# BurnhamG/PyTorch-ScalableFHVAE

Hardware: AMD Instinct MI355X
Metric: segments/sec + ELBO (nats/frame), (B,20,80) fbank (higher is better)
Workload: dtype bf16; 1 GPU; c3: fhvae.FHVAE 2x256 LSTM enc/dec, z1=z2=32, 28k-seq mu2 table, batch 2048; per-GPU batch 2048, T=20, F=80, full train step (fwd+loss+bwd+Adam), intended objective, mu_idx uniform; global_batch=2048, parallelism=single

## Files before the change

### pytorch-scalablefhvae_amd/csrc/wgrad.hip

```cpp
#include "wgrad.h"

#include <algorithm>
#include <cstdlib>
#include <type_traits>
#include <vector>

#include "gemm_core.h"

namespace fh {

constexpr int kWgThreads = 512, kWgBM = 256, kMaxWgProblems = FHVAE_WGRAD_MAX_PROBLEMS;

struct WgBf16 {
  using T = u16;
  using Frag = bf16x8;
  static constexpr int BK = 64, KB = 32;
  static constexpr bool kSetprio = true;
  static constexpr unsigned kOob = 0x40000000u;
  static constexpr int64_t kMaxBytes = 1LL << 30;
  static constexpr double kRate = 1.0e15;
  static __device__ __forceinline__ int swizzle(int pc, int row) { return (((pc >> 1) ^ (row & 7)) << 1) | (pc & 1); }
  static constexpr int kXor = 7, kSegShift = 5;
  static __device__ __forceinline__ int krow(int gq, int i) { return 4 * gq + (i >> 2); }
  static __device__ __forceinline__ int sub(int i) { return 8 * (i & 3); }
  template <int RB>
  static __device__ __forceinline__ Frag read(const char* a0) {
    typedef s16x4 __attribute__((address_space(3))) * lds_p;
    union {
      struct {
        s16x4 lo, hi;
      } s;
      bf16x8 v;
    } u;
    u.s.lo = __builtin_amdgcn_ds_read_tr16_b64_v4i16((lds_p)(a0));
    u.s.hi = __builtin_amdgcn_ds_read_tr16_b64_v4i16((lds_p)(a0 + 16 * RB));
    return u.v;
  }
  static __device__ __forceinline__ f32x4 mfma(Frag a, Frag b, f32x4 c) { return __builtin_amdgcn_mfma_f32_16x16x32_bf16(a, b, c, 0, 0, 0); }
};

struct WgF32 {
  using T = float;
  using Frag = float;
  static constexpr int BK = 32, KB = 4;
  static constexpr bool kSetprio = false;
  static constexpr unsigned kOob = 0x7ffffff0u;
  static constexpr int64_t kMaxBytes = 0x7ffffff0LL;
  static constexpr double kRate = 140.0e12;
  static __device__ __forceinline__ int swizzle(int pc, int row) { return (((pc >> 2) ^ (row & 3)) << 2) | (pc & 3); }
  static constexpr int kXor = 3, kSegShift = 6;
  static __device__ __forceinline__ int krow(int gq, int i) { return gq; }
  static __device__ __forceinline__ int sub(int i) { return i * 4; }
  template <int RB>
  static __device__ __forceinline__ Frag read(const char* a0) {
    return *(const float*)a0;
  }
  static __device__ __forceinline__ f32x4 mfma(Frag a, Frag b, f32x4 c) { return __builtin_amdgcn_mfma_f32_16x16x4f32(a, b, c, 0, 0, 0); }
};
template <class T>
using WgElem = std::conditional_t<std::is_same<T, u16>::value, WgBf16, WgF32>;

template <class E>
struct WgGroupT {
  int n;
  int base[kMaxWgProblems + 1];
  WgProblemT<typename E::T> p[kMaxWgProblems];
};

template <class E, int W>
struct WgImg {
  static constexpr int RB = W * (int)sizeof(typename E::T);
  static constexpr int BYTES = E::BK * RB;
  static constexpr int CPR = RB / 16;
  static constexpr int RPI = 1024 / RB;
  static constexpr int NI = BYTES / 1024 / 8;
};

typedef void __attribute__((address_space(3))) * lds_void_p;

template <class E, int W, int NI>
__device__ __forceinline__ void wg_dma_offsets(unsigned (&voff)[NI], unsigned ld_bytes, int wave, int lane) {
  using I = WgImg<E, W>;
#pragma unroll
  for (int q = 0; q < I::NI; ++q) {
    const int row = (wave * I::NI + q) * I::RPI + lane / I::CPR;
    const int pc = lane % I::CPR;
    voff[q] = (unsigned)row * ld_bytes + (unsigned)E::swizzle(pc, row) * 16u;
  }
}

template <class E, int W, int NI>
__device__ __forceinline__ void wg_issue(char* stage, __amdgpu_buffer_rsrc_t rs, const unsigned (&voff)[NI], unsigned kbase, int wave) {
  using I = WgImg<E, W>;
#pragma unroll
  for (int q = 0; q < I::NI; ++q)
    __builtin_amdgcn_raw_ptr_buffer_load_lds(rs, (lds_void_p)(stage + (wave * I::NI + q) * 1024), 16, voff[q] + kbase, 0, 0, 0);
}

template <class E, int BN>
__global__ __launch_bounds__(kWgThreads) void wgrad_kernel(WgGroupT<E> g) {
  using T = typename E::T;
  using IA = WgImg<E, kWgBM>;
  using IB = WgImg<E, BN>;
  constexpr int STAGE = IA::BYTES + IB::BYTES;
  constexpr int TM = 8, TN = BN / 64;
  constexpr int BK = E::BK, NJ = BK / E::KB;
  __shared__ __attribute__((aligned(1024))) char stage0[STAGE];
  __shared__ __attribute__((aligned(1024))) char stage1[STAGE];

  int wg = blockIdx.x;
  {
    const int nb = gridDim.x;
    if (nb >= 16) {
      const int q = nb >> 3, r = nb & 7, xcd = wg & 7;
      wg = (xcd < r ? xcd * (q + 1) : r * (q + 1) + (xcd - r) * q) + (wg >> 3);
    }
  }
  int pi = 0;
  while (pi + 1 < g.n && wg >= g.base[pi + 1]) ++pi;
  const WgProblemT<T>& p = g.p[pi];
  const int local = wg - g.base[pi];
  const int mt = local % p.m_tiles, nt = (local / p.m_tiles) % p.n_tiles, sp = local / (p.m_tiles * p.n_tiles);
  const int ks_total = (p.K + BK - 1) / BK;
  const int ks0 = sp * p.ksteps_per, ks1 = min(ks_total, ks0 + p.ksteps_per);
  if (ks0 >= ks1) return;
  const int m0 = mt * kWgBM, n0 = nt * BN;

  const int tid = threadIdx.x, lane = tid & 63, wave = tid >> 6;
  const int wm = wave >> 2, wn = wave & 3;
  const int gq = lane >> 4, i = lane & 15;

  constexpr unsigned ES = sizeof(T);
  const unsigned lda_b = (unsigned)p.lda * ES, ldb_b = (unsigned)p.ldb * ES;
  const __amdgpu_buffer_rsrc_t rsa =
      __builtin_amdgcn_make_buffer_rsrc(const_cast<T*>(p.A + m0), 0, (int)(((int64_t)p.K * p.lda - p.a_col0 - m0) * ES), 0x00020000);
  const __amdgpu_buffer_rsrc_t rsb =
      __builtin_amdgcn_make_buffer_rsrc(const_cast<T*>(p.B + n0), 0, (int)(((int64_t)p.K * p.ldb - n0) * ES), 0x00020000);
  unsigned va[IA::NI], vb[IB::NI];
  wg_dma_offsets<E, kWgBM>(va, lda_b, wave, lane);
  wg_dma_offsets<E, BN>(vb, ldb_b, wave, lane);

  const int kr = E::krow(gq, i), x = kr & E::kXor;
  int offa[TM], offb[TN];
#pragma unroll
  for (int tm = 0; tm < TM; ++tm) offa[tm] = kr * IA::RB + (((wm * 8 + tm) ^ x) << E::kSegShift) + E::sub(i);
#pragma unroll
  for (int tn = 0; tn < TN; ++tn) offb[tn] = kr * IB::RB + (((wn * TN + tn) ^ x) << E::kSegShift) + E::sub(i);

  f32x4 acc[TM][TN];
#pragma unroll
  for (int tm = 0; tm < TM; ++tm)
#pragma unroll
    for (int tn = 0; tn < TN; ++tn) acc[tm][tn] = f32x4{0.f, 0.f, 0.f, 0.f};

  auto kofs = [&](int ks, unsigned ld_b) __attribute__((always_inline)) -> unsigned { return (unsigned)(ks * BK) * ld_b; };
  auto compute = [&](const char* As, char* nxt, int ks_next) __attribute__((always_inline)) {
    const char* Bs = As + IA::BYTES;
#pragma unroll
    for (int j = 0; j < NJ; ++j) {
      typename E::Frag a[TM], b[TN];
#pragma unroll
      for (int tn = 0; tn < TN; ++tn) b[tn] = E::template read<IB::RB>(Bs + offb[tn] + j * E::KB * IB::RB);
#pragma unroll
      for (int tm = 0; tm < TM; ++tm) a[tm] = E::template read<IA::RB>(As + offa[tm] + j * E::KB * IA::RB);
      if (j == 0 || j == NJ / 2) {
        const bool in = ks_next < ks1;
        if (j == 0)
          wg_issue<E, kWgBM>(nxt, rsa, va, in ? kofs(ks_next, lda_b) : E::kOob, wave);
        else
          wg_issue<E, BN>(nxt + IA::BYTES, rsb, vb, in ? kofs(ks_next, ldb_b) : E::kOob, wave);
      }
      if (E::kSetprio) __builtin_amdgcn_s_setprio(1);
#pragma unroll
      for (int tm = 0; tm < TM; ++tm)
#pragma unroll
        for (int tn = 0; tn < TN; ++tn) acc[tm][tn] = E::mfma(a[tm], b[tn], acc[tm][tn]);
      if (E::kSetprio) __builtin_amdgcn_s_setprio(0);
    }
  };
  auto step = [&](const char* cur, char* nxt, int ks_next) __attribute__((always_inline)) {
    asm volatile("s_waitcnt vmcnt(0)" ::: "memory");
    __builtin_amdgcn_s_barrier();
    compute(cur, nxt, ks_next);
    __builtin_amdgcn_s_barrier();
  };
  wg_issue<E, kWgBM>(stage0, rsa, va, kofs(ks0, lda_b), wave);
  wg_issue<E, BN>(stage0 + IA::BYTES, rsb, vb, kofs(ks0, ldb_b), wave);
  for (int ks = ks0; ks < ks1; ks += 2) {
    step(stage0, stage1, ks + 1);
    step(stage1, stage0, ks + 2);
  }
  asm volatile("s_waitcnt vmcnt(0)" ::: "memory");

#pragma unroll
  for (int tm = 0; tm < TM; ++tm)
#pragma unroll
    for (int tn = 0; tn < TN; ++tn) {
      const int n = n0 + wn * (BN / 4) + tn * 16 + i;
#pragma unroll
      for (int r = 0; r < 4; ++r) {
        const int m = m0 + wm * 128 + tm * 16 + 4 * gq + r;
        if (m < p.M && n < p.N) {
          float* c = p.C + (int64_t)m * p.ldc + n;
          if (p.splitk == 1 && !p.shared_c)
            *c += acc[tm][tn][r];
          else
            atomicAdd(c, acc[tm][tn][r]);
        }
      }
    }
}

template __global__ void wgrad_kernel<WgBf16, 256>(WgGroupT<WgBf16>);
template __global__ void wgrad_kernel<WgBf16, 128>(WgGroupT<WgBf16>);
template __global__ void wgrad_kernel<WgF32, 256>(WgGroupT<WgF32>);
template __global__ void wgrad_kernel<WgF32, 128>(WgGroupT<WgF32>);

template <class T>
bool wgrad_eligible(const WgProblemT<T>& p) {
  using E = WgElem<T>;
  constexpr int64_t ES = sizeof(T);
  if (p.M <= 0 || p.N <= 0 || p.K <= 0 || !p.A || !p.B || !p.C) return false;
  if ((((uintptr_t)p.A) | ((uintptr_t)p.B)) & 15) return false;
  if ((p.lda % (16 / ES)) || (p.ldb % (16 / ES)) || p.lda < p.a_col0 + p.M || p.ldb < p.N || p.a_col0 < 0) return false;
  if ((int64_t)p.K * p.lda * ES >= E::kMaxBytes || (int64_t)p.K * p.ldb * ES >= E::kMaxBytes) return false;
  return true;
}

template <class T>
static void plan_launch(const WgProblemT<T>* ps, fhvae_wgrad_plan& l) {
  using E = WgElem<T>;
  int64_t tiles = 0, ks_max = 1;
  for (int k = 0; k < l.n; ++k) {
    const WgProblemT<T>& p = ps[l.p[k].which];
    tiles += fh_cdiv(p.M, kWgBM) * fh_cdiv(p.N, l.BN);
    ks_max = std::max<int64_t>(ks_max, fh_cdiv(p.K, E::BK));
  }
  const double t_step = 2.0 * kWgBM * l.BN * E::BK / (E::kRate / 256), tile_bytes = 4.0 * kWgBM * l.BN;
  int64_t sk = 1;
  double best = 1e30;
  for (int64_t c = 1; c <= 64 && c * 2 <= ks_max; ++c) {
    const double waves = (double)fh_cdiv(tiles * c, 256), steps = (double)fh_cdiv(ks_max, c) + 2.0;
    const double t = waves * steps * t_step + (c > 1 ? tiles * c * tile_bytes / 1.3e12 : 0.0);
    if (t < best) best = t, sk = c;
  }
  l.sk = (int)sk;
  for (int k = 0; k < l.n; ++k) {
    auto& q = l.p[k];
    const WgProblemT<T>& p = ps[q.which];
    q.m_tiles = (int)fh_cdiv(p.M, kWgBM);
    q.n_tiles = (int)fh_cdiv(p.N, l.BN);
    const int64_t ks_total = fh_cdiv(p.K, E::BK);
    int64_t s = sk;
    if (s > ks_total / 2) s = ks_total / 2;
    if (s < 1) s = 1;
    q.ksteps_per = (int)fh_cdiv(ks_total, s);
    q.splitk = (int)fh_cdiv(ks_total, q.ksteps_per);
    l.grid += q.m_tiles * q.n_tiles * q.splitk;
    for (int b = 0; b < l.n; ++b)
      if (b != k && ps[l.p[b].which].C == p.C) q.shared_c = 1;
  }
}

template <class T>
static int plan_wgrad(const WgProblemT<T>* ps, int n, fhvae_wgrad_plan* out, int cap) {
  if (n > 256) return FHVAE_ERR_LIMIT;
  for (int k = 0; k < n; ++k)
    if (!wgrad_eligible(ps[k])) return FHVAE_ERR_ALIGN;
  int launches = 0;
  for (const int BN : {256, 128}) {
    fhvae_wgrad_plan* l = nullptr;
    for (int k = 0; k < n; ++k) {
      if ((ps[k].N > 128) != (BN == 256)) continue;
// ... 100 lines not shown
```

### pytorch-scalablefhvae_amd/csrc/lstm.hip

```cpp
#include "gemm_launch.h"
#include "lstm_cell.h"
#include "lstm_cluster.h"
#include "lstm_point.h"
#include "wgrad.h"
#include <algorithm>
#include <vector>
#include "trace.h"
#include <cstdlib>
#include <type_traits>

namespace fh {

constexpr int kCH = 32;

struct GateRowMap {
  int H;
  __device__ __forceinline__ int64_t operator()(int n) const {
    int unit = (n >> 6) * 16 + (n & 15);
    int gate = (n & 63) >> 4;
    return unit < H ? (int64_t)gate * H + unit : -1;
  }
  __device__ __forceinline__ bool all_valid(int n0, int n) const { return ((n0 + n) >> 6) * 16 <= H; }
};

// ... 741 lines not shown
  };
  auto wgrad = [&](const void* a, int64_t lda, const void* b, int64_t ldb, int64_t Kc, float* c, int64_t ldc, int64_t Ncols) {
    GemmParams p = {};
    p.seg[0] = Seg{a, lda, 0, b, ldb, 0, (int)Kc, 0};
    p.M = (int)G;
    p.N = (int)Ncols;
    p.C = c;
    p.ldc = ldc;
    p.splitk = 0;
    p.mode = 1;
    return p;
  };
  auto flush = [&]() -> int {
    int e = FHVAE_OK;
    for (int i = 0; i < ng && !e; i += kMaxGroup) e = launch_gemm_group(grp + i, ng - i < kMaxGroup ? ng - i : kMaxGroup, d->dtype, st);
    ng = 0;
    return e;
  };
  for (int l = 0; l < L; ++l) {
    const T* dgl = dg + (int64_t)l * T_ * B * G;
    const T* hl = hs + (int64_t)l * T_ * B * H;
    int e;
    if (bd->dw_hh[l] && T_ > 1 && !wgrad_long(dgl + B * G, G, hl, H, (T_ - 1) * B, bd->dw_hh[l], H, H))
      grp[ng++] = wgrad(dgl + B * G, G, hl, H, (T_ - 1) * B, bd->dw_hh[l], H, H);
    if (bd->dw_ih[l]) {
      if (l > 0) {
        if (!wgrad_long(dgl, G, hs + (int64_t)(l - 1) * T_ * B * H, H, T_ * B, bd->dw_ih[l], H, H))
          grp[ng++] = wgrad(dgl, G, hs + (int64_t)(l - 1) * T_ * B * H, H, T_ * B, bd->dw_ih[l], H, H);
      } else {
        if (I > 0 && !wgrad_long(dgl, G, op.x, I, T_ * B, bd->dw_ih[0], K0, I))
          grp[ng++] = wgrad(dgl, G, op.x, I, T_ * B, bd->dw_ih[0], K0, I);
        if (Ic > 0) {
          GemmParams p = wgrad(bd->dgsum, G, d->xc, Ic, B, bd->dw_ih[0] + I, K0, Ic);
          if (fq) {
            fq->push_back(p);
          } else {
            e = launch_gemm(p, FHVAE_F32, st);
            if (e) return e;
          }
        }
      }
    }
    if (!pl.form) {
      if (l == 0 && Ic > 0 && bd->dgsum)
        e = launch_colsum(bd->dgsum, FHVAE_F32, G, bd->db_ih[l], bd->db_hh[l], B, G, st);
      else
        e = launch_colsum(dgl, d->dtype, G, bd->db_ih[l], bd->db_hh[l], T_ * B, G, st);
      if (e) return e;
    }
  }
  return flush();
}

static int lstm_dxc(const fhvae_lstm_bwd_desc* bd, hipStream_t st, bool zeroed) {
  const fhvae_lstm_desc* d = &bd->f;
  if (!bd->d_xc || d->Ic <= 0) return FHVAE_OK;
  const int64_t G = 4 * d->H, K0 = d->I + d->Ic;
  GemmParams p = {};
  p.seg[0] = Seg{bd->dgsum, G, 1, d->w_ih[0] + d->I, K0, 0, (int)G, 0};
  p.M = (int)d->B;
  p.N = (int)d->Ic;
  p.C = bd->d_xc;
  p.ldc = d->Ic;
  const int64_t tiles = fh_cdiv(d->B, 64) * fh_cdiv(d->Ic, 64);
  if (tiles <= 64 && G >= 512) {
    const int64_t n = d->B * d->Ic;
    if (!zeroed) hipLaunchKernelGGL(zero_f32_kernel, dim3((unsigned)fh_cdiv(n, 1024)), dim3(256), 0, st, bd->d_xc, n);
    p.mode = 2;
    int64_t sk = 256 / tiles;
    while (sk > 1 && G / sk < 128) sk >>= 1;
    p.splitk = (int)(sk < 4 ? 4 : sk > 16 ? 16 : sk);
  } else {
    p.splitk = 1;
  }
  return launch_gemm(p, FHVAE_F32, st);
}

template <typename T>
static int lstm_seq_bwd_t(const fhvae_lstm_bwd_desc* bd, const LstmPlan& pl, const Ops<T>& op, bool rec, bool par, hipStream_t st) {
  int e;
  if (rec) {
    e = lstm_bwd_impl<T>(bd, pl, op, st);
    if (e) return e;
    e = lstm_dxc(bd, st, pl.bwd_zeroes_dxc);
    if (e) return e;
  }
  if (!par) return FHVAE_OK;
  std::vector<WgProblemT<T>> wq;
  e = lstm_param_grads<T>(bd, pl, op, st, &wq);
  if (e) return e;
  return launch_wgrad(wq.data(), (int)wq.size(), st);
}

extern "C" int fhvae_lstm_seq_bwd(const fhvae_lstm_bwd_desc* bd, void* stream) {
  FH_CHECK_PTR(bd);
  const fhvae_lstm_desc* d = &bd->f;
  int e = check_desc(d);
  if (e) return e;
  FH_CHECK_PTR(bd->dgates);
  FH_CHECK_PTR(bd->dc);
  if (d->Ic > 0) FH_CHECK_PTR(bd->dgsum);
  if (bd->phase < 0 || bd->phase > 2) return FHVAE_ERR_SHAPE;
  const bool rec = bd->phase != 2, par = bd->phase != 1;
  if (rec && !bd->d_hs_top && !bd->d_hn) return FHVAE_ERR_NULL;
  hipStream_t st = (hipStream_t)stream;
  const LstmPlan pl = lstm_plan(d);
  if (d->dtype == FHVAE_F32) return lstm_seq_bwd_t<float>(bd, pl, ops_f32(d), rec, par, st);
  return lstm_seq_bwd_t<u16>(bd, pl, ops_bf16(d), rec, par, st);
}

static bool wg_from_desc(const fhvae_wgrad_desc* x, WgProblem& p) {
  if (!x || x->M <= 0 || x->N <= 0 || x->K <= 0 || x->M > INT32_MAX || x->N > INT32_MAX || x->K > INT32_MAX || x->a_col0 < 0 ||
      x->a_col0 > INT32_MAX)
    return false;
  p = WgProblem{};
  p.A = (const u16*)x->a, p.B = (const u16*)x->b, p.C = x->c;
  p.lda = x->lda, p.ldb = x->ldb, p.ldc = x->ldc;
  p.M = (int)x->M, p.N = (int)x->N, p.K = (int)x->K;
  p.a_col0 = (int)x->a_col0;
  return wgrad_eligible(p) && x->ldc >= x->N;
}

extern "C" int fhvae_wgrad_desc_ok(const fhvae_wgrad_desc* x) {
  WgProblem p;
  return wg_from_desc(x, p) ? 1 : 0;
}

extern "C" int fhvae_lstm_param_grads_multi(const fhvae_lstm_bwd_desc* const* bds, int n, const fhvae_wgrad_desc* extra, int n_extra,
                                            void* stream) {
  if (n < 0 || n_extra < 0) return FHVAE_ERR_SHAPE;
  if (n > 0) FH_CHECK_PTR(bds);
  if (n_extra > 0) FH_CHECK_PTR(extra);
  hipStream_t st = (hipStream_t)stream;
  std::vector<WgProblem> wq;
  for (int i = 0; i < n_extra; ++i) {
    WgProblem p;
    if (!wg_from_desc(extra + i, p)) return FHVAE_ERR_ALIGN;
    wq.push_back(p);
  }
  std::vector<GemmParams> fq;
  std::vector<WgProblem32> wq32;
  for (int i = 0; i < n; ++i) {
    const fhvae_lstm_bwd_desc* bd = bds[i];
    FH_CHECK_PTR(bd);
    const fhvae_lstm_desc* d = &bd->f;
    int e = check_desc(d);
    if (e) return e;
    FH_CHECK_PTR(bd->dgates);
    if (d->Ic > 0) FH_CHECK_PTR(bd->dgsum);
    if (d->dtype == FHVAE_F32) {
      e = lstm_param_grads<float>(bd, lstm_plan(d), ops_f32(d), st, &wq32);
    } else {
      e = lstm_param_grads<u16>(bd, lstm_plan(d), ops_bf16(d), st, &wq, &fq);
    }
    if (e) return e;
  }
  for (size_t i = 0; i < fq.size();) {
    size_t j = i;
    while (j < fq.size() && j - i < (size_t)kMaxGroup) {
      bool dup = false;
      for (size_t k = i; k < j; ++k) dup = dup || fq[k].C == fq[j].C;
      if (dup) break;
      ++j;
    }
    const int e = launch_gemm_group(fq.data() + i, (int)(j - i), FHVAE_F32, st);
    if (e) return e;
    i = j;
  }
// ... 7 lines not shown
```

### pytorch-scalablefhvae_amd/csrc/lstm_bwd_rs.hip

```cpp
#include <cstdlib>

#include "lstm_cluster_dev.h"
#include "lstm_point.h"
#include "trace.h"

namespace fh {

namespace {

constexpr int kH = 256, kG = 4 * kH, kHU = 64, kNU = 4;
constexpr int kKS = 8;

template <int RT>
__device__ __forceinline__ int rs_xoff(int par, int cluster, int src, int j, int wave, int rt) {
  return ((((((par * 64 + cluster) * kNU + src) * 3 + (j - 1)) * 4 + wave) * RT + rt) << 9);
}

template <int RT>
struct RsCfg {
  static constexpr int SMEM = RT * 16 * 512;
};

template <int RT, bool UM>
__global__ __launch_bounds__(kThreads) void lstm_bwd_layer_rs_kernel(ClBwd p) {
// ... 138 lines not shown
#pragma unroll
      for (int i = 0; i < 4; ++i) {
        const LstmPointBwd pt = lstm_point_bwd(dh[rt][i], ig[i], fg[i], gg[i], og[i], ccur[rt][i], cprev[rt][i], s > 0, dcreg[rt][i]);
        dcreg[rt][i] = pt.dc;
#pragma unroll
        for (int g = 0; g < 4; ++g) dp[g][i] = pt.dp[g];
      }
      ccur[rt] = cprev[rt];
      const bool live = row[rt] < rend;
#pragma unroll
      for (int g = 0; g < 4; ++g) {
        if (live) dgs[rt][g] += dp[g];
        dpk[rt][g] = pack4(dp[g]);
        *(uint2*)(Img + wbase[g & 1] + (g >> 1) * 256 + rt * 8192) = dpk[rt][g];
      }
    }
    asm volatile("s_waitcnt lgkmcnt(0)\n\ts_barrier" ::: "memory");
    CL_TLOG(s * 8 + 3);
    if (s + 1 < T) {
      f32x4 acc[RT][kNU];
#pragma unroll
      for (int rt = 0; rt < RT; ++rt)
#pragma unroll
        for (int j = 0; j < kNU; ++j) acc[rt][j] = f32x4{0.f, 0.f, 0.f, 0.f};
      bf16x8 bfrag[2][RT];
      auto ifrag = [&](int ks, int buf) {
#pragma unroll
        for (int rt = 0; rt < RT; ++rt)
          bfrag[buf][rt] = __builtin_bit_cast(bf16x8, *(const uint4*)(Img + ibase[ks & 3] + (ks >> 2) * 256 + rt * 8192));
      };
      ifrag(0, 0);
      __builtin_amdgcn_sched_group_barrier(0x100, RT, 0);
#pragma unroll
      for (int ks = 0; ks < kKS; ++ks) {
        if (ks + 1 < kKS) ifrag(ks + 1, (ks + 1) & 1);
#pragma unroll
        for (int j = 0; j < kNU; ++j)
#pragma unroll
          for (int rt = 0; rt < RT; ++rt) acc[rt][j] = __builtin_amdgcn_mfma_f32_16x16x32_bf16(wreg[ks][j], bfrag[ks & 1][rt], acc[rt][j], 0, 0, 0);
        if (ks + 1 < kKS) {
          __builtin_amdgcn_sched_group_barrier(0x008, 1, 0);
          __builtin_amdgcn_sched_group_barrier(0x100, RT, 0);
          __builtin_amdgcn_sched_group_barrier(0x008, RT * kNU - 1, 0);
        } else {
          __builtin_amdgcn_sched_group_barrier(0x008, RT * kNU, 0);
        }
      }
#pragma unroll
      for (int rt = 0; rt < RT; ++rt) {
        own[rt] = acc[rt][0];
#pragma unroll
        for (int j = 1; j < kNU; ++j)
          *(uint2*)((char*)p.xch + rs_xoff<RT>(s & 1, cluster, me, j, wave, rt) + lane * 8) = pack4(acc[rt][j]);
      }
    }
    auto img_chunk = [&](int i) -> uint4 {
      const int c = (wave * RT * 2 + i) * 64 + lane;
      return *(const uint4*)(Img + kc_off<32>(c >> 5, c & 31));
    };
    const uint4 v0 = img_chunk(0), v1 = img_chunk(1), v2 = RT > 1 ? img_chunk(2) : uint4{0u, 0u, 0u, 0u},
                v3 = RT > 1 ? img_chunk(3) : uint4{0u, 0u, 0u, 0u};
    CL_TLOG(s * 8 + 4);
    if (s + 1 < T) cluster_publish(flags, me, ep0 + (unsigned)(s + 1));
    else __syncthreads();
    CL_TLOG(s * 8 + 5);
    auto dg_store = [&](int i, const uint4& v) {
      const int c = (wave * RT * 2 + i) * 64 + lane;
      const int rw = r0 + (c >> 5), cc = c & 31;
      if (rw < rend) {
        u16* dst = p.dg + ((int64_t)t * B + rw) * G + (cc >> 3) * H + u0 + (cc & 7) * 8;
        if (nt)
          __builtin_nontemporal_store(u32x4v{v.x, v.y, v.z, v.w}, (u32x4v*)dst);
        else
          *(uint4*)dst = v;
      }
    };
    dg_store(0, v0);
    dg_store(1, v1);
    if constexpr (RT > 1) {
      dg_store(2, v2);
      dg_store(3, v3);
    }
  }
  if (p.d_xc_zero && me == 0 && wave == 0) {
#pragma unroll
    for (int rt = 0; rt < RT; ++rt)
      if (row[rt] < rend)
        for (int c = q; c < p.Ic; c += 4) p.d_xc_zero[(int64_t)row[rt] * p.Ic + c] = 0.f;
  }
#pragma unroll
  for (int g = 0; g < 4; ++g) {
    f32x4 vs = f32x4{0.f, 0.f, 0.f, 0.f};
#pragma unroll
    for (int rt = 0; rt < RT; ++rt) {
      vs += dgs[rt][g];
      if (p.dgsum && row[rt] < rend) *(f32x4*)(p.dgsum + (int64_t)row[rt] * G + g * H + uq) = dgs[rt][g];
    }
    if (p.db_ih[0] || p.db_hh[0]) db_reduce_add(vs, p.db_ih[0], p.db_hh[0], g * H + uq, lane);
  }
  CL_TLOG((T - 1) * 8 + 7);
}

template <int RT>
int launch_rs(const ClBwd& p, hipStream_t st) {
  if (p.gates_um)
    hipLaunchKernelGGL((lstm_bwd_layer_rs_kernel<RT, true>), dim3(kGrid), dim3(kThreads), RsCfg<RT>::SMEM, st, p);
  else
    hipLaunchKernelGGL((lstm_bwd_layer_rs_kernel<RT, false>), dim3(kGrid), dim3(kThreads), RsCfg<RT>::SMEM, st, p);
  return fh_launch_status();
}

}

int cluster_bwd_layer_rs(const ClBwd& p, hipStream_t st) {
  if (p.NU != kNU || p.Mc > 32 || p.Mc % 16 != 0) return FHVAE_ERR_SHAPE;
  return p.Mc <= 16 ? launch_rs<1>(p, st) : launch_rs<2>(p, st);
}

}
```

### pytorch-scalablefhvae_amd/csrc/lstm_cluster.h

```cpp
#pragma once
#include "common.h"

namespace fh {

constexpr int kSyncStatus = 0;
constexpr int kSyncSticky = 2;
constexpr int kSyncFlags = 64;
constexpr int kSyncXcdCnt = kSyncFlags + 64 * 32;
constexpr int kSyncXcdStride = 32;
constexpr int kSyncWordsUsed = 3072;
constexpr int kSeqEpochs = 4096;

constexpr int64_t kRsXchElems = 2LL * 64 * 4 * 3 * 4 * 2 * 256;

struct ClusterWeights {
  const u16* w_ih[FHVAE_MAX_LAYERS];
  const u16* w_hh[FHVAE_MAX_LAYERS];
  const u16* w_ih_t[FHVAE_MAX_LAYERS];
  const u16* w_hh_t[FHVAE_MAX_LAYERS];
  u16* xch;
  const u16* x_fold;
  const u16* xc_fold;
};

struct LstmPlan {
  int form;
  bool big, big_shape;
  bool fold;
  bool xc_in;
  bool bwd_rs;
  bool fwd_wr;
  bool bwd_zeroes_dxc;
  bool needs_ws_below;
  bool wgrad;
  bool tlog;
  struct Geo {
    int NU, NC;
    int64_t chunk;
  } fwd, bwd;
};
LstmPlan lstm_plan(const fhvae_lstm_desc* d);

int cluster_fwd(const fhvae_lstm_desc* d, const LstmPlan& pl, const ClusterWeights& w, hipStream_t st);
int cluster_bwd(const fhvae_lstm_bwd_desc* bd, const LstmPlan& pl, const ClusterWeights& w, hipStream_t st);

}
```

### pytorch-scalablefhvae_amd/csrc/lstm_cluster.hip

```cpp
#include "lstm_cluster_dev.h"
#include "lstm_point.h"

#include <cstdlib>
#include <cstring>
#include <type_traits>

#include "gemm_core.h"
#include "gemm_launch.h"
#include "proj.h"
#include "trace.h"


namespace fh {

constexpr int kRing = 4;
constexpr int kPanel = 4096;

template <int ROWS, int CH, class RowMap>
__device__ __forceinline__ void glds_wave_panel(char* lds, const u16* base, int64_t ld, int k0, const RowMap& rm, int row_base,
                                                int lane) {
  constexpr int RPI = 64 / CH;
  constexpr int SW = CH >= 16 ? 15 : CH - 1;
  static_assert(ROWS * CH * 16 == kPanel && ROWS % RPI == 0, "panel shape");
#pragma unroll
// ... 1020 lines not shown
        dcreg[i] = pt.dc;
#pragma unroll
        for (int g = 0; g < 4; ++g) dp[g][i] = pt.dp[g];
      }
      ccur = cprev;
      if (row < rend) {
#pragma unroll
        for (int g = 0; g < 4; ++g) dgs[g] += dp[g];
      }
      if (row < rend) {
#pragma unroll
        for (int g = 0; g < 4; ++g) {
          dpk[g] = pack4(dp[g]);
          *(uint2*)(p.xch + xch_off(s & 1, kp, L, KS, (g * H + uq) >> 5, B, row) + (uq & 31)) = dpk[g];
        }
      }
    }
    CL_TLOG(s * 8 + 3);
    if (s + 1 < nsteps) cluster_publish(flags, me, ep0 + (unsigned)(s + 1));
    CL_TLOG(s * 8 + 4);
    if (act && row < rend) {
      u16* go = p.dg + (((int64_t)kp * T + t) * B + row) * G + uq;
#pragma unroll
      for (int g = 0; g < 4; ++g) *(uint2*)(go + g * H) = dpk[g];
    }
  }
  if (p.dgsum && kp == 0 && row < rend) {
#pragma unroll
    for (int g = 0; g < 4; ++g) *(f32x4*)(p.dgsum + (int64_t)row * G + g * H + uq) = dgs[g];
    if (p.d_xc_zero && uq == 0)
      for (int c = 0; c < p.Ic; ++c) p.d_xc_zero[(int64_t)row * p.Ic + c] = 0.f;
  }
  if (epi && (p.db_ih[kp] || p.db_hh[kp])) {
#pragma unroll
    for (int g = 0; g < 4; ++g) db_reduce_add(dgs[g], p.db_ih[kp], p.db_hh[kp], g * H + uq, lane);
  }
}

static bool device_ok() {
  static int ok = -1;
  if (ok < 0) {
    int dev = 0;
    hipDeviceProp_t pr;
    ok = 0;
    if (hipGetDevice(&dev) == hipSuccess && hipGetDeviceProperties(&pr, dev) == hipSuccess)
      ok = (strncmp(pr.gcnArchName, "gfx950", 6) == 0 && pr.multiProcessorCount == kGrid) ? 1 : 0;
  }
  return ok == 1;
}

static void cluster_rows(int64_t nrows, int NC, int* Mc, int* RB) {
  int64_t m = (nrows + NC - 1) / NC;
  m = (m + 15) / 16 * 16;
  *Mc = (int)m;
  *RB = m <= 16 ? 16 : m <= 32 ? 32 : m <= 64 ? 64 : 128;
}

LstmPlan lstm_plan(const fhvae_lstm_desc* d) {
  const int64_t B = d->B, T = d->T, I = d->I, Ic = d->Ic, H = d->H;
  LstmPlan p = {};
  p.wgrad = !getenv("FHVAE_NO_WGRAD");
  const bool persistent = !getenv("FHVAE_NO_CLUSTER") && d->dtype == FHVAE_BF16 && d->lp && (H == 256 || H == 128) && d->L <= 2 &&
                          T + d->L < kSeqEpochs && B <= 131072 &&
                          device_ok();
  if (!persistent) {
    const char* ev = getenv("FHVAE_BIG_CELLS");
    const int want = ev ? atoi(ev) : -1, es = d->dtype == FHVAE_BF16 ? 2 : 4, epc = 16 / es;
    p.big = want >= 0 ? want != 0 : (B / 128) * (H / 64) >= (d->dtype == FHVAE_F32 ? 64 : 96);
    p.big_shape = !(B % 128 || H % 64 || I % epc || Ic % epc) && B * 4 * H * 4 < (1LL << 31) && (int64_t)d->L * H * B * 4 < (1LL << 31) &&
                  4 * H * (I + Ic > H ? I + Ic : H) * es < (1LL << 30);
    return p;
  }
  const int NU = (int)H / 16, NC = kGrid / NU;
  int Mc, RB;
  cluster_rows(B < (int64_t)NC * 128 ? B : (int64_t)NC * 128, NC, &Mc, &RB);
  p.form = RB <= 32 ? 2 : 1;
  p.tlog = getenv("FHVAE_CLUSTER_TLOG") != nullptr;
  p.fold = I > 0 && I % 8 == 0 && I <= 128 && (I + Ic) % 8 == 0 && !getenv("FHVAE_NO_FOLD");
  p.xc_in = Ic > 0 && Ic % 8 == 0 && Ic <= 128 && I % 8 == 0 && (I == 0 || p.fold) && !getenv("FHVAE_NO_XC_FOLD");
  p.bwd_rs = p.form == 1 && H == 256 && !getenv("FHVAE_NO_RS");
  p.fwd_wr = p.bwd_rs && d->L == 2 && !getenv("FHVAE_NO_FWD_WR") && (I == 0 || p.fold) && (Ic == 0 || p.xc_in) &&
             2 * T * B * H * 2 < (1LL << 31) && T * B * I * 2 < (1LL << 31) && I + Ic > 0;
  p.bwd_zeroes_dxc = p.bwd_rs || p.form == 2;
  p.needs_ws_below = p.form == 1 && d->L >= 2;
  p.fwd = p.fwd_wr ? LstmPlan::Geo{8, kGrid / 8, (int64_t)(kGrid / 8) * 64} : LstmPlan::Geo{NU, NC, (int64_t)NC * 128};
  const int NUb = (int)H / (p.form == 2 ? 16 : p.bwd_rs ? 64 : 32);
  p.bwd = LstmPlan::Geo{NUb, kGrid / NUb, (int64_t)(kGrid / NUb) * (p.bwd_rs ? 32 : 128)};
  return p;
}

template <auto kernel, class P>
static int launch_cl(const P& p, int grid, int threads, int smem, hipStream_t st) {
  static bool attr = false;
  if (!attr) {
    hipError_t e = hipFuncSetAttribute((const void*)kernel, hipFuncAttributeMaxDynamicSharedMemorySize, smem);
    if (e != hipSuccess) return (int)e;
    attr = true;
  }
  hipLaunchKernelGGL(kernel, dim3(grid), dim3(threads), smem, st, p);
  return fh_launch_status();
}

template <class P>
static int chunk_params(P& p, const fhvae_lstm_desc* d, const LstmPlan& pl, const LstmPlan::Geo& g, const ClusterWeights& w, int64_t row0) {
  const int64_t nrows = d->B - row0 < g.chunk ? d->B - row0 : g.chunk;
  int RB;
  cluster_rows(nrows, g.NC, &p.Mc, &RB);
  p.B = (int)d->B;
  p.T = (int)d->T;
  p.NU = g.NU;
  p.row0 = (int)row0;
  p.nrows = (int)nrows;
  p.sync = (unsigned*)d->lp;
  p.xch = w.xch;
  p.tlog = pl.tlog ? (unsigned long long*)((char*)d->lp + FHVAE_LSTM_SYNC_BYTES * 3 / 4) : nullptr;
  return RB;
}

template <bool kSave, int H, int L>
static int launch_fwd_save(const ClFwd& p, int RB, hipStream_t st) {
  constexpr int KS_SMEM = (2 * L - 1) * 64 * (H / 8) * 16 + 4 * L * 4 * 1024 + 16;
  switch (RB) {
    case 16: return launch_cl<lstm_fwd_ksplit_kernel<H, L, 16, kSave>>(p, kGrid, kThreads, KS_SMEM, st);
    case 32: return launch_cl<lstm_fwd_ksplit_kernel<H, L, 32, kSave>>(p, kGrid, kThreads, KS_SMEM, st);
    case 64: return launch_cl<lstm_fwd_cluster_kernel<H, L, 64, kSave>>(p, kGrid, kThreads, ClFwdCfg<H, L, 64>::SMEM, st);
    default: return launch_cl<lstm_fwd_cluster_kernel<H, L, 128, kSave>>(p, kGrid, kThreads, ClFwdCfg<H, L, 128>::SMEM, st);
  }
}
template <int H, int L>
static int launch_fwd(const ClFwd& p, int RB, hipStream_t st) {
  return p.gates ? launch_fwd_save<true, H, L>(p, RB, st) : launch_fwd_save<false, H, L>(p, RB, st);
}

int cluster_fwd(const fhvae_lstm_desc* d, const LstmPlan& pl, const ClusterWeights& w, hipStream_t st) {
  const int H = (int)d->H, L = d->L;
  for (int64_t row0 = 0; row0 < d->B; row0 += pl.fwd.chunk) {
    ClFwd p = {};
    const int RB = chunk_params(p, d, pl, pl.fwd, w, row0);
    for (int l = 0; l < L; ++l) {
      p.w_ih[l] = w.w_ih[l];
      p.w_hh[l] = w.w_hh[l];
      p.b_ih[l] = d->b_ih[l];
      p.b_hh[l] = d->b_hh[l];
    }
    if (w.x_fold) {
      p.x = w.x_fold;
      p.w_ih0 = w.w_ih[0];
      p.I = (int)d->I;
      p.K0 = (int)(d->I + d->Ic);
      p.pre = d->Ic > 0 ? d->pre : nullptr;
      p.pre_tstride = 0;
    } else {
      p.pre = d->pre;
      p.pre_tstride = d->I > 0 ? d->B * 4 * d->H : 0;
    }
    if (w.xc_fold) {
      p.xcv = w.xc_fold;
      p.Ic = (int)d->Ic;
      p.w_ih0 = w.w_ih[0];
      p.I = (int)d->I;
      p.K0 = (int)(d->I + d->Ic);
      p.pre = nullptr;
      p.pre_tstride = 0;
    }
    p.hs = (u16*)d->hs;
    p.cs = d->gates ? d->cs : nullptr;
// ... 1 lines not shown
    p.hs_top_f32 = d->hs_top_f32;
    p.hn = d->hn;
    p.hn_lp = (u16*)d->hn_lp;
    p.il = 1;
    p.gates_um = pl.fwd_wr;
    double fl = 0;
    for (int l = 0; l < L; ++l) fl += 2.0 * p.nrows * 4 * H * ((l > 0 ? d->T * H : 0) + (d->T - 1) * (double)H);
    const int ts = trace_begin(st, kTraceFwdCell, fl);
    int e;
    if (pl.fwd_wr)
      e = cluster_fwd_wr(p, st);
    else if (H == 256)
      e = L == 1 ? launch_fwd<256, 1>(p, RB, st) : launch_fwd<256, 2>(p, RB, st);
    else
      e = L == 1 ? launch_fwd<128, 1>(p, RB, st) : launch_fwd<128, 2>(p, RB, st);
    trace_end(st, ts);
    if (e) return e;
  }
  return FHVAE_OK;
}

template <int H, int L>
static int launch_bwd(const ClBwd& p, int RB, hipStream_t st) {
  constexpr int SMEM = (2 * L - 1) * 16 * (4 * H / 8) * 16 + 4 * L * 1024 + 16;
  return RB <= 16 ? launch_cl<lstm_bwd_ksplit_kernel<H, L, 16>>(p, kGrid, kThreads, SMEM, st)
                  : launch_cl<lstm_bwd_ksplit_kernel<H, L, 32>>(p, kGrid, kThreads, SMEM, st);
}

template <int H, int RB>
static int launch_bwd_layer(const ClBwd& p, hipStream_t st) {
  using CF = ClLayerCfg<H, RB, 32>;
  constexpr bool HW = RB <= 64 && CF::SMEM_HW <= 163840;
  return launch_cl<lstm_bwd_layer_kernel<H, RB, 32, HW>>(p, kGrid, HW ? kThreads + 64 : kThreads, HW ? CF::SMEM_HW : CF::SMEM, st);
}
template <int H>
static int launch_bwd_layer_rb(const ClBwd& p, int RB, hipStream_t st) {
  switch (RB) {
    case 16: return launch_bwd_layer<H, 16>(p, st);
    case 32: return launch_bwd_layer<H, 32>(p, st);
    case 64: return launch_bwd_layer<H, 64>(p, st);
    default: return launch_bwd_layer<H, 128>(p, st);
  }
}

static int cluster_bwd_layers(const fhvae_lstm_bwd_desc* bd, const LstmPlan& pl, const ClusterWeights& w, hipStream_t st) {
  const fhvae_lstm_desc* d = &bd->f;
  const int H = (int)d->H, L = d->L;
  const bool rs = pl.bwd_rs;
  const int64_t B = d->B, T = d->T, G = 4 * H;
  for (int l = L - 1; l >= 0; --l) {
    if (l < L - 1) {
      const u16* dg_up = (const u16*)bd->dgates + (int64_t)(l + 1) * T * B * G;
      int e;
      if (rs && proj_eligible(dg_up, G, w.w_ih_t[l + 1], G, bd->ws_below, H, T * B, H, G)) {
        e = launch_proj(dg_up, G, w.w_ih_t[l + 1], G, bd->ws_below, H, nullptr, T * B, H, G, st);
      } else {
        GemmParams g = {};
        g.seg[0] = Seg{dg_up, G, 1, w.w_ih_t[l + 1], G, 1, (int)G, 0};
        g.M = (int)(T * B);
        g.N = H;
        g.C = bd->ws_below;
        g.ldc = H;
        g.splitk = 1;
        e = launch_gemm(g, FHVAE_BF16, st);
      }
      if (e) return e;
    }
    for (int64_t row0 = 0; row0 < B; row0 += pl.bwd.chunk) {
      ClBwd p = {};
      const int RB = chunk_params(p, d, pl, pl.bwd, w, row0);
      p.w_hh_t[0] = w.w_hh_t[l];
      p.gates = (const u16*)d->gates + (int64_t)l * T * B * G;
      p.cs = d->cs + (int64_t)l * T * B * H;
      p.d_hs_top = l == L - 1 ? bd->d_hs_top : bd->ws_below;
      p.d_hn = bd->d_hn ? bd->d_hn + (int64_t)l * H : nullptr;
      p.hn_ld = L * H;
      p.dg = (u16*)bd->dgates + (int64_t)l * T * B * G;
      p.dgsum = (l == 0 && d->Ic > 0) ? bd->dgsum : nullptr;
      p.db_ih[0] = bd->db_ih[l];
      p.db_hh[0] = bd->db_hh[l];
      p.tlog_slot = l == L - 1;
      p.nt = 1;
      p.gates_um = pl.fwd_wr;
      if (rs && l == 0 && bd->d_xc && d->Ic > 0) p.d_xc_zero = bd->d_xc, p.Ic = (int)d->Ic;
      const int ts = trace_begin(st, kTraceBwdCell, 2.0 * p.nrows * H * (T - 1) * 4.0 * H);
      const int e = rs ? cluster_bwd_layer_rs(p, st) : (H == 256 ? launch_bwd_layer_rb<256>(p, RB, st) : launch_bwd_layer_rb<128>(p, RB, st));
      trace_end(st, ts);
      if (e) return e;
    }
  }
  return FHVAE_OK;
}

int cluster_bwd(const fhvae_lstm_bwd_desc* bd, const LstmPlan& pl, const ClusterWeights& w, hipStream_t st) {
  const fhvae_lstm_desc* d = &bd->f;
  const int H = (int)d->H, L = d->L;
  if (pl.form == 1) {
    if (pl.needs_ws_below && !bd->ws_below) return FHVAE_ERR_NULL;
    return cluster_bwd_layers(bd, pl, w, st);
  }
  for (int64_t row0 = 0; row0 < d->B; row0 += pl.bwd.chunk) {
    ClBwd p = {};
    const int RB = chunk_params(p, d, pl, pl.bwd, w, row0);
    for (int l = 0; l < L; ++l) {
      p.w_ih_t[l] = w.w_ih_t[l];
      p.w_hh_t[l] = w.w_hh_t[l];
    }
    p.gates = (const u16*)d->gates;
    p.cs = d->cs;
    p.d_hs_top = bd->d_hs_top;
    p.d_hn = bd->d_hn;
    p.hn_ld = L * H;
    p.dg = (u16*)bd->dgates;
    p.dgsum = d->Ic > 0 ? bd->dgsum : nullptr;
    if (bd->d_xc && d->Ic > 0) p.d_xc_zero = bd->d_xc, p.Ic = (int)d->Ic;
    for (int l = 0; l < L; ++l) p.db_ih[l] = bd->db_ih[l], p.db_hh[l] = bd->db_hh[l];
    double fl = 0;
    for (int l = 0; l < L; ++l) fl += 2.0 * p.nrows * H * ((l < L - 1 ? d->T * 4.0 * H : 0) + (d->T - 1) * 4.0 * H);
    const int ts = trace_begin(st, kTraceBwdCell, fl);
    int e;
    if (H == 256)
      e = L == 1 ? launch_bwd<256, 1>(p, RB, st) : launch_bwd<256, 2>(p, RB, st);
    else
      e = L == 1 ? launch_bwd<128, 1>(p, RB, st) : launch_bwd<128, 2>(p, RB, st);
    trace_end(st, ts);
    if (e) return e;
  }
  return FHVAE_OK;
}

}
```

### pytorch-scalablefhvae_amd/csrc/lstm_cluster_dev.h

```cpp
#pragma once
#include "lstm_cluster.h"

#include "gemm_core.h"

#define RLX_AGENT __ATOMIC_RELAXED, __HIP_MEMORY_SCOPE_AGENT

namespace fh {

constexpr unsigned kSpinLimit = 1u << 21;
constexpr int kGrid = 256;
constexpr int kSc1 = 16;

__device__ __forceinline__ unsigned xcc_id() {
  unsigned v;
  asm volatile("s_getreg_b32 %0, hwreg(HW_REG_XCC_ID)" : "=s"(v));
  return v & 0xf;
}

__device__ __forceinline__ void cluster_give_up(unsigned* sync, unsigned code) {
  __hip_atomic_fetch_or(sync + kSyncStatus, code, RLX_AGENT);
  const unsigned long long a = (unsigned long long)__hip_atomic_load(sync + kSyncSticky, RLX_AGENT) |
                               ((unsigned long long)__hip_atomic_load(sync + kSyncSticky + 1, RLX_AGENT) << 32);
  if (a) __hip_atomic_fetch_or((unsigned*)a, code, RLX_AGENT);
}
// ... 37 lines not shown
}

struct ClRowMap {
  int r0, rlast;
  __device__ __forceinline__ int64_t operator()(int r) const {
    const int x = r0 + r;
    return x < rlast ? x : rlast;
  }
};
struct ClGateMap {
  int H, u0;
  __device__ __forceinline__ int64_t operator()(int n) const { return (int64_t)(n >> 4) * H + u0 + (n & 15); }
};
struct ClUnitMap {
  int u0;
  __device__ __forceinline__ int64_t operator()(int n) const { return u0 + n; }
};


__device__ __forceinline__ int cl_goff(int uq) { return (uq >> 4) * 64 + ((uq >> 2) & 3) * 8; }
__device__ __forceinline__ void cl_load_gates(const u16* row_base, int uq, uint2 (&g)[4]) {
  const uint4 a = *(const uint4*)(row_base + cl_goff(uq)), b = *(const uint4*)(row_base + cl_goff(uq) + 32);
  g[0] = uint2{a.x, a.y}, g[1] = uint2{a.z, a.w}, g[2] = uint2{b.x, b.y}, g[3] = uint2{b.z, b.w};
}
__device__ __forceinline__ void cl_store_gates(u16* row_base, int uq, const uint2 (&g)[4]) {
  *(uint4*)(row_base + cl_goff(uq)) = uint4{g[0].x, g[0].y, g[1].x, g[1].y};
  *(uint4*)(row_base + cl_goff(uq) + 32) = uint4{g[2].x, g[2].y, g[3].x, g[3].y};
}

#define CL_TLOG(slot)                                                                                      \
  do {                                                                                                     \
    if (tl && tid == 0) tl[(slot)] = wall_clock64();                                                        \
  } while (0)

typedef unsigned int u32x4 __attribute__((ext_vector_type(4)));
typedef unsigned int u32x2 __attribute__((ext_vector_type(2)));

__device__ __forceinline__ __amdgpu_buffer_rsrc_t make_rsrc(const void* p) {
  return __builtin_amdgcn_make_buffer_rsrc(const_cast<void*>(p), 0, 0x7fffffff, 0x00020000);
}
__device__ __forceinline__ uint4 load_sc1(__amdgpu_buffer_rsrc_t rs, int64_t byte_off) {
  const u32x4 v = __builtin_amdgcn_raw_buffer_load_b128(rs, (int)byte_off, 0, kSc1);
  return uint4{v.x, v.y, v.z, v.w};
}


__device__ __forceinline__ void db_reduce_add(f32x4 v, float* db_a, float* db_b, int col, int lane) {
#pragma unroll
  for (int off = 1; off < 16; off <<= 1)
#pragma unroll
    for (int i = 0; i < 4; ++i) v[i] += __shfl_xor(v[i], off, 64);
  const int i = lane & 15;
  if (i < 4) {
    const float s = i == 0 ? v[0] : i == 1 ? v[1] : i == 2 ? v[2] : v[3];
    if (db_a) atomicAdd(db_a + col + i, s);
    if (db_b) atomicAdd(db_b + col + i, s);
  }
}

struct ClBwd {
  int B, T, NU, Mc;
  int row0, nrows;
  const u16* w_ih_t[2];
  const u16* w_hh_t[2];
  const u16* gates;
  const float* cs;
  const float* d_hs_top;
  const float* d_hn;
  int hn_ld;
  u16* dg;
  float* dgsum;
  float* db_ih[2];
  float* db_hh[2];
  u16* xch;
  unsigned* sync;
  unsigned long long* tlog;
  const u16* dg_above;
  const u16* w_above_t;
  int gates_um;
  int tlog_slot;
  int nt;
  float* d_xc_zero;
  int Ic;
};

__device__ __forceinline__ f32x4 unpack4(uint2 v) {
  return f32x4{bf2f((u16)(v.x & 0xffff)), bf2f((u16)(v.x >> 16)), bf2f((u16)(v.y & 0xffff)), bf2f((u16)(v.y >> 16))};
}
__device__ __forceinline__ uint2 pack4(const f32x4& v) {
  return uint2{(uint32_t)f2bf(v[0]) | ((uint32_t)f2bf(v[1]) << 16), (uint32_t)f2bf(v[2]) | ((uint32_t)f2bf(v[3]) << 16)};
}

struct ClFwd {
  int B, T, NU, Mc;
  int row0, nrows;
  const u16* w_ih[2];
  const u16* w_hh[2];
  const float* b_ih[2];
  const float* b_hh[2];
  const float* pre;
  int64_t pre_tstride;
  const u16* x;
  const u16* w_ih0;
  int I, K0;
  u16* hs;
  float* cs;
  u16* gates;
  float* hs_top_f32;
  float* hn;
  u16* hn_lp;
  u16* xch;
  unsigned* sync;
  unsigned long long* tlog;
  int il;
  const u16* xcv;
  int Ic;
  int gates_um;
};

int cluster_fwd_wr(const ClFwd& p, hipStream_t st);

int cluster_bwd_layer_rs(const ClBwd& p, hipStream_t st);

}
```

Before: 1.286 million segments/s.

## Deepen wgrad LDS pipeline to a three-stage ring with partial vmcnt waits

```diff
diff --git a/pytorch-scalablefhvae_amd/csrc/wgrad.hip b/pytorch-scalablefhvae_amd/csrc/wgrad.hip
--- a/pytorch-scalablefhvae_amd/csrc/wgrad.hip
+++ b/pytorch-scalablefhvae_amd/csrc/wgrad.hip
@@ -76,6 +76,17 @@
   static constexpr int NI = BYTES / 1024 / 8;
 };
 
+constexpr int kWgLds = 160 * 1024;
+template <class E, int BN>
+struct WgRing {
+  static constexpr int A_BYTES = WgImg<E, kWgBM>::BYTES, B_BYTES = WgImg<E, BN>::BYTES;
+  static constexpr bool fits(int nsa, int nsb) { return nsa * A_BYTES + nsb * B_BYTES <= kWgLds; }
+  static constexpr bool kDeep = !(std::is_same<E, WgF32>::value && BN == 256);
+  static constexpr int NSA = kDeep && fits(3, 2) ? 3 : 2;
+  static constexpr int NSB = kDeep && fits(3, 3) ? 3 : 2;
+  static_assert(fits(NSA, NSB) && NSB <= NSA && NSA <= NSB + 1, "ring depths");
+};
+
 typedef void __attribute__((address_space(3))) * lds_void_p;
 
 template <class E, int W, int NI>
@@ -102,11 +113,24 @@
   using T = typename E::T;
   using IA = WgImg<E, kWgBM>;
   using IB = WgImg<E, BN>;
-  constexpr int STAGE = IA::BYTES + IB::BYTES;
+  using R = WgRing<E, BN>;
   constexpr int TM = 8, TN = BN / 64;
   constexpr int BK = E::BK, NJ = BK / E::KB;
-  __shared__ __attribute__((aligned(1024))) char stage0[STAGE];
-  __shared__ __attribute__((aligned(1024))) char stage1[STAGE];
+  constexpr int PA = IA::NI, PB = IB::NI;
+  constexpr int NSA = R::NSA, NSB = R::NSB, LA = NSA - 1, LB = NSB - 1;
+  constexpr int PERIOD = NSA == NSB ? NSA : NSA * NSB;
+  constexpr bool kTwoStage = NSA == 2 && NSB == 2;
+  static_assert(IA::BYTES % 8192 == 0 && IB::BYTES % 8192 == 0, "every wave issues the same number of 1-KB pieces");
+  __shared__ __attribute__((aligned(1024))) char sa0[IA::BYTES + (kTwoStage ? IB::BYTES : 0)];
+  __shared__ __attribute__((aligned(1024))) char sa1[IA::BYTES + (kTwoStage ? IB::BYTES : 0)];
+  __shared__ __attribute__((aligned(1024))) char sa2[NSA > 2 ? IA::BYTES : 1024];
+  __shared__ __attribute__((aligned(1024))) char sb0[kTwoStage ? 1024 : IB::BYTES];
+  __shared__ __attribute__((aligned(1024))) char sb1[kTwoStage ? 1024 : IB::BYTES];
+  __shared__ __attribute__((aligned(1024))) char sb2[NSB > 2 ? IB::BYTES : 1024];
+  auto slot_a = [&](int i) __attribute__((always_inline)) -> char* { return i == 0 ? sa0 : i == 1 ? sa1 : sa2; };
+  auto slot_b = [&](int i) __attribute__((always_inline)) -> char* {
+    return kTwoStage ? (i == 0 ? sa0 : sa1) + IA::BYTES : i == 0 ? sb0 : i == 1 ? sb1 : sb2;
+  };
 
   int wg = blockIdx.x;
   {
@@ -153,22 +177,39 @@
 #pragma unroll
     for (int tn = 0; tn < TN; ++tn) acc[tm][tn] = f32x4{0.f, 0.f, 0.f, 0.f};
 
-  auto kofs = [&](int ks, unsigned ld_b) __attribute__((always_inline)) -> unsigned { return (unsigned)(ks * BK) * ld_b; };
-  auto compute = [&](const char* As, char* nxt, int ks_next) __attribute__((always_inline)) {
-    const char* Bs = As + IA::BYTES;
+  const int nsteps = ks1 - ks0;
+  auto issue_a = [&](char* st, int s) __attribute__((always_inline)) {
+    wg_issue<E, kWgBM>(st, rsa, va, s < nsteps ? (unsigned)((ks0 + s) * BK) * lda_b : E::kOob, wave);
+  };
+  auto issue_b = [&](char* st, int s) __attribute__((always_inline)) {
+    wg_issue<E, BN>(st, rsb, vb, s < nsteps ? (unsigned)((ks0 + s) * BK) * ldb_b : E::kOob, wave);
+  };
+  constexpr bool A_FIRST = NSA == NSB;
+  constexpr int WAIT = A_FIRST ? (LA - 1) * (PA + PB) : PA + (LB - 1) * (PA + PB);
+  auto compute = [&](const char* As, const char* Bs, char* na, char* nb, int s) __attribute__((always_inline)) {
+    int oa[TM], ob[TN];
+#pragma unroll
+    for (int tm = 0; tm < TM; ++tm) {
+      oa[tm] = offa[tm];
+      if (!kTwoStage) asm volatile("" : "+v"(oa[tm]));
+    }
+#pragma unroll
+    for (int tn = 0; tn < TN; ++tn) {
+      ob[tn] = offb[tn];
+      if (!kTwoStage) asm volatile("" : "+v"(ob[tn]));
+    }
 #pragma unroll
     for (int j = 0; j < NJ; ++j) {
       typename E::Frag a[TM], b[TN];
 #pragma unroll
-      for (int tn = 0; tn < TN; ++tn) b[tn] = E::template read<IB::RB>(Bs + offb[tn] + j * E::KB * IB::RB);
-#pragma unroll
-      for (int tm = 0; tm < TM; ++tm) a[tm] = E::template read<IA::RB>(As + offa[tm] + j * E::KB * IA::RB);
+      for (int tn = 0; tn < TN; ++tn) b[tn] = E::template read<IB::RB>(Bs + ob[tn] + j * E::KB * IB::RB);
+#pragma unroll
+      for (int tm = 0; tm < TM; ++tm) a[tm] = E::template read<IA::RB>(As + oa[tm] + j * E::KB * IA::RB);
       if (j == 0 || j == NJ / 2) {
-        const bool in = ks_next < ks1;
-        if (j == 0)
-          wg_issue<E, kWgBM>(nxt, rsa, va, in ? kofs(ks_next, lda_b) : E::kOob, wave);
+        if ((j == 0) == A_FIRST)
+          issue_a(na, s + LA);
         else
-          wg_issue<E, BN>(nxt + IA::BYTES, rsb, vb, in ? kofs(ks_next, ldb_b) : E::kOob, wave);
+          issue_b(nb, s + LB);
       }
       if (E::kSetprio) __builtin_amdgcn_s_setprio(1);
 #pragma unroll
@@ -178,17 +219,26 @@
       if (E::kSetprio) __builtin_amdgcn_s_setprio(0);
     }
   };
-  auto step = [&](const char* cur, char* nxt, int ks_next) __attribute__((always_inline)) {
-    asm volatile("s_waitcnt vmcnt(0)" ::: "memory");
+#pragma unroll
+  for (int v = -LA; v < 0; ++v) {
+    if (!A_FIRST && v + LB >= 0) issue_b(slot_b(v + LB), v + LB);
+    issue_a(slot_a(v + LA), v + LA);
+    if (A_FIRST) issue_b(slot_b(v + LB), v + LB);
+  }
+  auto step = [&](int i, int s) __attribute__((always_inline)) {
+    asm volatile("s_waitcnt vmcnt(%0)" ::"n"(WAIT) : "memory");
     __builtin_amdgcn_s_barrier();
-    compute(cur, nxt, ks_next);
-    __builtin_amdgcn_s_barrier();
+    compute(slot_a(i % NSA), slot_b(i % NSB), slot_a((i + LA) % NSA), slot_b((i + LB) % NSB), s);
+    if (kTwoStage) __builtin_amdgcn_s_barrier();
   };
-  wg_issue<E, kWgBM>(stage0, rsa, va, kofs(ks0, lda_b), wave);
-  wg_issue<E, BN>(stage0 + IA::BYTES, rsb, vb, kofs(ks0, ldb_b), wave);
-  for (int ks = ks0; ks < ks1; ks += 2) {
-    step(stage0, stage1, ks + 1);
-    step(stage1, stage0, ks + 2);
+  int s = 0;
+  for (; s + PERIOD <= nsteps; s += PERIOD)
+#pragma unroll
+    for (int i = 0; i < PERIOD; ++i) step(i, s + i);
+#pragma unroll
+  for (int i = 0; i < PERIOD - 1; ++i) {
+    if (s + i >= nsteps) break;
+    step(i, s + i);
   }
   asm volatile("s_waitcnt vmcnt(0)" ::: "memory");
 
```

After: 1.286 million segments/s, median of 2. About the same (-0.0%).

## Fold constant-input gradient dxc into LSTM backward recurrent kernel epilogue

Applied to the files above, without the earlier changes.

```diff
diff --git a/pytorch-scalablefhvae_amd/csrc/lstm.hip b/pytorch-scalablefhvae_amd/csrc/lstm.hip
--- a/pytorch-scalablefhvae_amd/csrc/lstm.hip
+++ b/pytorch-scalablefhvae_amd/csrc/lstm.hip
@@ -847,8 +847,10 @@
   if (rec) {
     e = lstm_bwd_impl<T>(bd, pl, op, st);
     if (e) return e;
-    e = lstm_dxc(bd, st, pl.bwd_zeroes_dxc);
-    if (e) return e;
+    if (!pl.bwd_folds_dxc) {
+      e = lstm_dxc(bd, st, pl.bwd_zeroes_dxc);
+      if (e) return e;
+    }
   }
   if (!par) return FHVAE_OK;
   std::vector<WgProblemT<T>> wq;
diff --git a/pytorch-scalablefhvae_amd/csrc/lstm_bwd_rs.hip b/pytorch-scalablefhvae_amd/csrc/lstm_bwd_rs.hip
--- a/pytorch-scalablefhvae_amd/csrc/lstm_bwd_rs.hip
+++ b/pytorch-scalablefhvae_amd/csrc/lstm_bwd_rs.hip
@@ -244,7 +244,64 @@
       dg_store(3, v3);
     }
   }
-  if (p.d_xc_zero && me == 0 && wave == 0) {
+  f32x4 ms[RT];
+#pragma unroll
+  for (int i = 0; i < RT; ++i) ms[i] = f32x4{0.f, 0.f, 0.f, 0.f};
+  if (p.d_xc) {
+    const int Ic = p.Ic;
+    f32x4 xacc[RT][4];
+#pragma unroll
+    for (int rt = 0; rt < RT; ++rt)
+#pragma unroll
+      for (int ct = 0; ct < 4; ++ct) xacc[rt][ct] = f32x4{0.f, 0.f, 0.f, 0.f};
+#pragma unroll
+    for (int ct = 0; ct < 4; ++ct) {
+      if (ct * 16 < Ic) {
+        const int col = ct * 16 + r;
+        const float* wp = p.w_xc + (col < Ic ? col : Ic - 1);
+        float bv[4][4];
+#pragma unroll
+        for (int g = 0; g < 4; ++g)
+#pragma unroll
+          for (int j = 0; j < 4; ++j) {
+            const float v = wp[(int64_t)(g * H + uq + j) * p.ldw_xc];
+            bv[g][j] = col < Ic ? v : 0.f;
+          }
+#pragma unroll
+        for (int g = 0; g < 4; ++g)
+#pragma unroll
+          for (int j = 0; j < 4; ++j)
+#pragma unroll
+            for (int rt = 0; rt < RT; ++rt) xacc[rt][ct] = __builtin_amdgcn_mfma_f32_16x16x4f32(dgs[rt][g][j], bv[g][j], xacc[rt][ct], 0, 0, 0);
+      }
+    }
+    float* S = (float*)Img;
+    constexpr int HS = RT * 16 * 64;
+    auto xsum = [&](bool add) {
+      float* sh = S + (wave & 1) * HS;
+#pragma unroll
+      for (int rt = 0; rt < RT; ++rt)
+#pragma unroll
+        for (int ct = 0; ct < 4; ++ct)
+#pragma unroll
+          for (int v = 0; v < 4; ++v) {
+            float* e = sh + (rt * 16 + 4 * q + v) * 64 + ct * 16 + r;
+            *e = add ? *e + xacc[rt][ct][v] : xacc[rt][ct][v];
+          }
+    };
+    if (wave < 2) xsum(false);
+    __syncthreads();
+    if (wave >= 2) xsum(true);
+    __syncthreads();
+#pragma unroll
+    for (int i = 0; i < RT; ++i) ms[i] = *(const f32x4*)(S + (tid + 256 * i) * 4) + *(const f32x4*)(S + HS + (tid + 256 * i) * 4);
+    const int par = (T - 1) & 1;
+    if (me != 0) {
+#pragma unroll
+      for (int i = 0; i < RT; ++i) *(f32x4*)((char*)p.xch + rs_xoff<RT>(par, cluster, me, 1, 0, 0) + (tid + 256 * i) * 16) = ms[i];
+    }
+    cluster_publish(flags, me, ep0 + (unsigned)T);
+  } else if (p.d_xc_zero && me == 0 && wave == 0) {
 #pragma unroll
     for (int rt = 0; rt < RT; ++rt)
       if (row[rt] < rend)
@@ -259,6 +316,28 @@
       if (p.dgsum && row[rt] < rend) *(f32x4*)(p.dgsum + (int64_t)row[rt] * G + g * H + uq) = dgs[rt][g];
     }
     if (p.db_ih[0] || p.db_hh[0]) db_reduce_add(vs, p.db_ih[0], p.db_hh[0], g * H + uq, lane);
+  }
+  if (p.d_xc && me == 0) {
+    const int Ic = p.Ic, par = (T - 1) & 1;
+    if (!cluster_wait(p.sync, flags, kNU, ep0 + (unsigned)T)) return;
+    u32x4 pv[RT][3];
+#pragma unroll
+    for (int m = 1; m < kNU; ++m)
+#pragma unroll
+      for (int i = 0; i < RT; ++i)
+        pv[i][m - 1] = __builtin_amdgcn_raw_buffer_load_b128(x_rs, rs_xoff<RT>(par, cluster, m, 1, 0, 0) + (tid + 256 * i) * 16, 0, kSc1);
+#pragma unroll
+    for (int i = 0; i < RT; ++i) {
+      f32x4 v = ms[i];
+#pragma unroll
+      for (int m = 0; m < 3; ++m) v += __builtin_bit_cast(f32x4, pv[i][m]);
+      const int pc = tid + 256 * i, rw = r0 + (pc >> 4), c0 = (pc & 15) * 4;
+      if (rw < rend) {
+#pragma unroll
+        for (int k = 0; k < 4; ++k)
+          if (c0 + k < Ic) p.d_xc[(int64_t)rw * Ic + c0 + k] = v[k];
+      }
+    }
   }
   CL_TLOG((T - 1) * 8 + 7);
 }
diff --git a/pytorch-scalablefhvae_amd/csrc/lstm_cluster.h b/pytorch-scalablefhvae_amd/csrc/lstm_cluster.h
--- a/pytorch-scalablefhvae_amd/csrc/lstm_cluster.h
+++ b/pytorch-scalablefhvae_amd/csrc/lstm_cluster.h
@@ -31,6 +31,7 @@
   bool bwd_rs;
   bool fwd_wr;
   bool bwd_zeroes_dxc;
+  bool bwd_folds_dxc;
   bool needs_ws_below;
   bool wgrad;
   bool tlog;
diff --git a/pytorch-scalablefhvae_amd/csrc/lstm_cluster.hip b/pytorch-scalablefhvae_amd/csrc/lstm_cluster.hip
--- a/pytorch-scalablefhvae_amd/csrc/lstm_cluster.hip
+++ b/pytorch-scalablefhvae_amd/csrc/lstm_cluster.hip
@@ -1126,6 +1126,7 @@
   p.fwd_wr = p.bwd_rs && d->L == 2 && !getenv("FHVAE_NO_FWD_WR") && (I == 0 || p.fold) && (Ic == 0 || p.xc_in) &&
              2 * T * B * H * 2 < (1LL << 31) && T * B * I * 2 < (1LL << 31) && I + Ic > 0;
   p.bwd_zeroes_dxc = p.bwd_rs || p.form == 2;
+  p.bwd_folds_dxc = p.bwd_rs && Ic > 0 && Ic <= 64 && T >= 2 && !getenv("FHVAE_NO_DXC_FOLD");
   p.needs_ws_below = p.form == 1 && d->L >= 2;
   p.fwd = p.fwd_wr ? LstmPlan::Geo{8, kGrid / 8, (int64_t)(kGrid / 8) * 64} : LstmPlan::Geo{NU, NC, (int64_t)NC * 128};
   const int NUb = (int)H / (p.form == 2 ? 16 : p.bwd_rs ? 64 : 32);
@@ -1293,7 +1294,13 @@
       p.tlog_slot = l == L - 1;
       p.nt = 1;
       p.gates_um = pl.fwd_wr;
-      if (rs && l == 0 && bd->d_xc && d->Ic > 0) p.d_xc_zero = bd->d_xc, p.Ic = (int)d->Ic;
+      if (rs && l == 0 && bd->d_xc && d->Ic > 0) {
+        p.Ic = (int)d->Ic;
+        if (pl.bwd_folds_dxc)
+          p.d_xc = bd->d_xc, p.w_xc = d->w_ih[0] + d->I, p.ldw_xc = (int)(d->I + d->Ic);
+        else
+          p.d_xc_zero = bd->d_xc;
+      }
       const int ts = trace_begin(st, kTraceBwdCell, 2.0 * p.nrows * H * (T - 1) * 4.0 * H);
       const int e = rs ? cluster_bwd_layer_rs(p, st) : (H == 256 ? launch_bwd_layer_rb<256>(p, RB, st) : launch_bwd_layer_rb<128>(p, RB, st));
       trace_end(st, ts);
diff --git a/pytorch-scalablefhvae_amd/csrc/lstm_cluster_dev.h b/pytorch-scalablefhvae_amd/csrc/lstm_cluster_dev.h
--- a/pytorch-scalablefhvae_amd/csrc/lstm_cluster_dev.h
+++ b/pytorch-scalablefhvae_amd/csrc/lstm_cluster_dev.h
@@ -143,6 +143,9 @@
   int nt;
   float* d_xc_zero;
   int Ic;
+  float* d_xc;
+  const float* w_xc;
+  int ldw_xc;
 };
 
 __device__ __forceinline__ f32x4 unpack4(uint2 v) {
```

Result: faster. 1.285 million segments/s before, 1.301 million segments/s after (median of 6 runs) (+1.2%).
